# lab-emi/CleanUMamba

Hardware: AMD Instinct MI355X
Metric: audio samples/sec/node (train step, E8, 10s@16kHz) (higher is better)
Workload: dtype f16

## Files before the change

### cleanumamba_amd/csrc/gemm.hip

```cpp
#include <stdlib.h>
#include <type_traits>
#include "common.h"

namespace cum {

typedef __attribute__((ext_vector_type(8))) __bf16 bf16x8;
typedef __attribute__((ext_vector_type(8))) _Float16 f16x8;
typedef __attribute__((ext_vector_type(4))) float f32x4;
typedef __attribute__((ext_vector_type(4))) unsigned u32x4;

enum { EPI_BIAS = 0, EPI_RELU = 1, EPI_GLU = 2, EPI_MASK = 3, EPI_GLU_BWD = 4 };

struct GemmParams {
  const void *A, *W;
  const float *bias;
  const void *res;
  void *out;
  void *aux;
  const void *aux2;
  int64_t lda, ldw, ldc, ldr, ldz, ldy;
  int gate_only;
  int allow_split_k;
  int mask_bits;
  int M, N, K;
  int pitch, valid;
  int n_store;
  int64_t zero_head, zero_tail;
  int rows_epilogue;
  int group_m;
};

template <typename T>
struct Elem;
template <>
struct Elem<float> {
  static constexpr int EPC = 4;
  static __device__ __forceinline__ float to_f(float v) { return v; }
  static __device__ __forceinline__ float from_f(float v) { return v; }
};
template <>
struct Elem<__bf16> {
  static constexpr int EPC = 8;
  static __device__ __forceinline__ float to_f(__bf16 v) { return (float)v; }
  static __device__ __forceinline__ __bf16 from_f(float v) { return (__bf16)v; }
};

template <>
struct Elem<f16> {
  static constexpr int EPC = 8;
  static __device__ __forceinline__ float to_f(f16 v) { return (float)v; }
  static __device__ __forceinline__ f16 from_f(float v) { return (f16)v; }
};

template <typename T>
// ... 815 lines not shown
    __builtin_amdgcn_s_setprio(0);
    asm volatile("s_waitcnt lgkmcnt(0)"
                 : "+v"(af[0][4]), "+v"(af[0][5]), "+v"(af[0][6]), "+v"(af[0][7]), "+v"(af[1][4]), "+v"(af[1][5]),
                   "+v"(af[1][6]), "+v"(af[1][7]) : : "memory");
    asm volatile("s_barrier" ::: "memory");
    const bool early = more && wr == 0, late = more && wr != 0;
    if (early) {
      CUM_STAGE(0, kt + 2, par);
      CUM_STAGE(1, kt + 2, par);
    }
    __builtin_amdgcn_s_setprio(1);
    CUM_QUAD(1, 0);
    __builtin_amdgcn_s_setprio(0);
    __builtin_amdgcn_sched_barrier(0);
    if (late) {
      CUM_STAGE(0, kt + 2, par);
      CUM_STAGE(1, kt + 2, par);
    }
    CUM_DSR(wf[0][0], w0, 4096);  CUM_DSR(wf[0][1], w0, 6144);  CUM_DSR(wf[1][0], w1, 4096);  CUM_DSR(wf[1][1], w1, 6144);
    asm volatile("s_waitcnt lgkmcnt(0)" : "+v"(wf[0][0]), "+v"(wf[0][1]), "+v"(wf[1][0]), "+v"(wf[1][1]) : : "memory");
    asm volatile("s_barrier" ::: "memory");
    if (early) {
      CUM_STAGE(2, kt + 2, par);
      CUM_STAGE(3, kt + 2, par);
    }
    __builtin_amdgcn_s_setprio(1);
    CUM_QUAD(1, 2);
    __builtin_amdgcn_s_setprio(0);
    __builtin_amdgcn_sched_barrier(0);
    if (late) {
      CUM_STAGE(2, kt + 2, par);
      CUM_STAGE(3, kt + 2, par);
    }
    __builtin_amdgcn_s_setprio(1);
    CUM_QUAD(0, 2);
    __builtin_amdgcn_s_setprio(0);
  }
#undef CUM_HALFQ
#undef CUM_DSR
#undef CUM_QUAD
#undef CUM_STAGE
  asm volatile("s_barrier" ::: "memory");
  nt_epilogue_any<T, EPI, 2, 1>(p, acc, bv, m0, n0, 2 * wr, wc, lane,
                                reinterpret_cast<unsigned char *>(lds_all) + wave * nt_rows_lds(EPI));
}

#endif

template <typename T, int EPI>
__global__ __launch_bounds__(512) void gemm_nt9_kernel(const GemmParams p) {
  static_assert(sizeof(T) == 2, "16-bit element types only");
  constexpr int EPC = 8, BK = 64;
  constexpr int UNIT = 128 * 8;
  __shared__ uint4 lds_all[2 * 4 * UNIT];

  const int tid = threadIdx.x, lane = tid & 63;
  const int wave = uniform(tid >> 6);
  const int wr = wave >> 2, wc = wave & 3;
  const int g = lane >> 4, r = lane & 15;
  const int NB = (p.N + 255) / 256;
  const int xcd = blockIdx.x & 7, local = blockIdx.x >> 3;
  const int per = p.group_m * NB, grp = local / per, within = local - grp * per;
  const int left = (int)gridDim.x / (8 * NB) - grp * p.group_m;
  const int gm = left < p.group_m ? left : p.group_m;
  const int m_tile = (grp * p.group_m + within % gm) * 8 + xcd;
  const int n0 = (within / gm) * 256;
  const int m0 = m_tile * 256;
  if (m0 >= p.M) return;
  if (blockIdx.x == 0) {
    T *o = static_cast<T *>(p.out);
    T *x = (EPI != EPI_GLU && EPI != EPI_GLU_BWD && !(EPI == EPI_RELU && p.mask_bits)) ? static_cast<T *>(p.aux) : nullptr;
    for (int64_t i = threadIdx.x; i < p.zero_head; i += 512) {
      o[-1 - i] = Elem<T>::from_f(0.f);
      if (x) x[-1 - i] = Elem<T>::from_f(0.f);
    }
    const int64_t tail0 = (int64_t)p.M * p.ldc, tailx = (int64_t)p.M * p.ldz;
    for (int64_t i = threadIdx.x; i < p.zero_tail; i += 512) {
      o[tail0 + i] = Elem<T>::from_f(0.f);
      if (x) x[tailx + i] = Elem<T>::from_f(0.f);
    }
  }
  const T *A = static_cast<const T *>(p.A);
  const T *W = static_cast<const T *>(p.W);
  const T *src[4][2];
#pragma unroll
  for (int u = 0; u < 4; ++u)
#pragma unroll
    for (int it = 0; it < 2; ++it) {
      const int pos = it * 512 + tid;
      const int row = pos >> 3, cphys = pos & 7;
      const int clog = cphys ^ (row & 7);
      if (u < 2) {
        int am = m0 + 128 * u + row;
        am = am < p.M ? am : p.M - 1;
        src[u][it] = A + (int64_t)am * p.lda + clog * EPC;
      } else {
        int wn_ = n0 + 128 * (u - 2) + row;
        wn_ = wn_ < p.N ? wn_ : p.N - 1;
        src[u][it] = W + (int64_t)wn_ * p.ldw + clog * EPC;
      }
    }
  typedef __attribute__((address_space(3))) void *lds_ptr;
  typedef const __attribute__((address_space(1))) void *glb_ptr;
#define CUM_STAGE(u, kt, par)                                                                                   \
  do {                                                                                                          \
    _Pragma("unroll") for (int it = 0; it < 2; ++it)                                                           \
      __builtin_amdgcn_global_load_lds((glb_ptr)(src[u][it] + (kt) * BK),                                      \
                                       (lds_ptr)(&lds_all[((par) * 4 + (u)) * UNIT + it * 512 + wave * 64]), 16, 0, 0); \
  } while (0)

  f32x4 acc[2][4][4];
#pragma unroll
  for (int h = 0; h < 2; ++h)
#pragma unroll
    for (int i = 0; i < 4; ++i)
#pragma unroll
      for (int j = 0; j < 4; ++j) acc[h][i][j] = f32x4{0.f, 0.f, 0.f, 0.f};
  float bv[4][4];
  nt_load_bias(p, n0, wc, g, bv);

  const int nk = p.K / BK;
#pragma unroll
  for (int u = 0; u < 4; ++u) CUM_STAGE(u, 0, 0);
  if (nk > 1) {
#pragma unroll
    for (int u = 0; u < 4; ++u) CUM_STAGE(u, 1, 1);
  }
  const unsigned lds0 = (unsigned)(uintptr_t)(lds_ptr)lds_all;
  unsigned aA[2], aW[2];
#pragma unroll
  for (int ks = 0; ks < 2; ++ks) {
    const int cl = ks * 4 + g;
    aA[ks] = lds0 + (unsigned)((wr * UNIT + r * 8 + (cl ^ (r & 7))) * 16);
    aW[ks] = lds0 + (unsigned)(((2 + (wc >> 1)) * UNIT + ((wc & 1) * 64 + r) * 8 + (cl ^ (r & 7))) * 16);
  }
#define CUM_DSR(dst, addr, off) asm volatile("ds_read_b128 %0, %1 offset:" #off : "=v"(dst) : "v"(addr) : "memory")
#ifdef CUM_NT9_TIMING_NO_W_READS
#define CUM_DSRW(dst, addr, off) asm volatile("" : "=v"(dst) : "v"(addr))
#else
#define CUM_DSRW(dst, addr, off) CUM_DSR(dst, addr, off)
#endif
#define CUM_BAR()                               \
  do {                                          \
    __builtin_amdgcn_sched_barrier(0);          \
    asm volatile("s_barrier" ::: "memory");     \
    __builtin_amdgcn_sched_barrier(0);          \
  } while (0)
#define CUM_HALFQ(h, nlo, ks)                                                                                  \
  do {                                                                                                         \
    _Pragma("unroll") for (int ni = 0; ni < 2; ++ni)                                                           \
      _Pragma("unroll") for (int mi = 0; mi < 4; ++mi) {                                                       \
        if constexpr (__is_same(T, f16))                                                                       \
          acc[h][(nlo) + ni][mi] = __builtin_amdgcn_mfma_f32_16x16x32_f16(                                     \
              __builtin_bit_cast(f16x8, wf[ks][ni]), __builtin_bit_cast(f16x8, af[ks][4 * (h) + mi]),          \
              acc[h][(nlo) + ni][mi], 0, 0, 0);                                                                \
        else                                                                                                   \
          acc[h][(nlo) + ni][mi] = __builtin_amdgcn_mfma_f32_16x16x32_bf16(                                    \
              __builtin_bit_cast(bf16x8, wf[ks][ni]), __builtin_bit_cast(bf16x8, af[ks][4 * (h) + mi]),        \
              acc[h][(nlo) + ni][mi], 0, 0, 0);                                                                \
      }                                                                                                        \
  } while (0)
#define CUM_QUAD(h, nlo)                 \
  do {                                   \
    __builtin_amdgcn_s_setprio(1);       \
    CUM_HALFQ(h, nlo, 0);                \
    CUM_HALFQ(h, nlo, 1);                \
    __builtin_amdgcn_s_setprio(0);       \
  } while (0)

  if (nk > 1) asm volatile("s_waitcnt vmcnt(8)" ::: "memory");
  else asm volatile("s_waitcnt vmcnt(0)" ::: "memory");
  CUM_BAR();
  if (wr != 0) CUM_BAR();
  u32x4 af[2][8], wf[2][2];
  for (int kt = 0; kt < nk; ++kt) {
    const int par = kt & 1;
    const unsigned pb = (unsigned)par * (4 * UNIT * 16);
    const unsigned a0 = aA[0] + pb, a1 = aA[1] + pb, w0 = aW[0] + pb, w1 = aW[1] + pb;
    const bool more1 = kt + 1 < nk, more2 = kt + 2 < nk;
    CUM_DSRW(wf[0][0], w0, 0);    CUM_DSRW(wf[0][1], w0, 2048);
    CUM_DSR(af[0][0], a0, 0);     CUM_DSR(af[0][1], a0, 2048);  CUM_DSR(af[0][2], a0, 4096);  CUM_DSR(af[0][3], a0, 6144);
    CUM_DSRW(wf[1][0], w1, 0);    CUM_DSRW(wf[1][1], w1, 2048);
    CUM_DSR(af[1][0], a1, 0);     CUM_DSR(af[1][1], a1, 2048);  CUM_DSR(af[1][2], a1, 4096);  CUM_DSR(af[1][3], a1, 6144);
    if (wr == 0 && kt >= 1 && more1) {
      CUM_STAGE(2, kt + 1, par ^ 1);
      CUM_STAGE(3, kt + 1, par ^ 1);
    }
    CUM_BAR();
    asm volatile("s_waitcnt lgkmcnt(0)"
                 : "+v"(wf[0][0]), "+v"(wf[0][1]), "+v"(wf[1][0]), "+v"(wf[1][1]), "+v"(af[0][0]), "+v"(af[0][1]),
                   "+v"(af[0][2]), "+v"(af[0][3]), "+v"(af[1][0]), "+v"(af[1][1]), "+v"(af[1][2]), "+v"(af[1][3]) : : "memory");
    CUM_QUAD(0, 0);
    CUM_BAR();
    CUM_DSR(af[0][4], a0, 8192);  CUM_DSR(af[0][5], a0, 10240); CUM_DSR(af[0][6], a0, 12288); CUM_DSR(af[0][7], a0, 14336);
    CUM_DSR(af[1][4], a1, 8192);  CUM_DSR(af[1][5], a1, 10240); CUM_DSR(af[1][6], a1, 12288); CUM_DSR(af[1][7], a1, 14336);
    CUM_BAR();
    asm volatile("s_waitcnt lgkmcnt(0)"
                 : "+v"(af[0][4]), "+v"(af[0][5]), "+v"(af[0][6]), "+v"(af[0][7]), "+v"(af[1][4]), "+v"(af[1][5]),
                   "+v"(af[1][6]), "+v"(af[1][7]) : : "memory");
    CUM_QUAD(1, 0);
    CUM_BAR();
    CUM_DSRW(wf[0][0], w0, 4096); CUM_DSRW(wf[0][1], w0, 6144); CUM_DSRW(wf[1][0], w1, 4096); CUM_DSRW(wf[1][1], w1, 6144);
    if (more2) {
      CUM_STAGE(0, kt + 2, par);
      if (wr != 0) CUM_STAGE(1, kt + 2, par);
    }
    CUM_BAR();
    asm volatile("s_waitcnt lgkmcnt(0)" : "+v"(wf[0][0]), "+v"(wf[0][1]), "+v"(wf[1][0]), "+v"(wf[1][1]) : : "memory");
    CUM_QUAD(1, 2);
    CUM_BAR();
    if (wr == 0) {
      if (more2) CUM_STAGE(1, kt + 2, par);
    } else {
      if (more1) {
        if (more2) asm volatile("s_waitcnt vmcnt(4)" ::: "memory");
        else asm volatile("s_waitcnt vmcnt(0)" ::: "memory");
      }
      if (more2) {
        CUM_STAGE(2, kt + 2, par);
        CUM_STAGE(3, kt + 2, par);
      }
    }
    CUM_BAR();
    CUM_QUAD(0, 2);
    if (wr == 0 && more1) {
      if (more2) asm volatile("s_waitcnt vmcnt(4)" ::: "memory");
      else asm volatile("s_waitcnt vmcnt(0)" ::: "memory");
    }
    CUM_BAR();
  }
  if (wr == 0) CUM_BAR();
#undef CUM_HALFQ
#undef CUM_DSRW
#undef CUM_DSR
#undef CUM_QUAD
#undef CUM_STAGE
#undef CUM_BAR
  asm volatile("s_barrier" ::: "memory");
  nt_epilogue_any<T, EPI, 2, 1>(p, acc, bv, m0, n0, 2 * wr, wc, lane,
                                reinterpret_cast<unsigned char *>(lds_all) + wave * nt_rows_lds(EPI));
}

template <typename T, int EPI>
__global__ __launch_bounds__(512) void gemm_nt_ring_kernel(const GemmParams p) {
  static_assert(sizeof(T) == 2, "16-bit element types only");
#ifndef CUM_RING_NST
#define CUM_RING_NST 3
#endif
  constexpr int EPC = 8, BK = 64, BM = 128, BN = 256, NST = CUM_RING_NST;
  static_assert(NST == 2 || NST == 3, "two or three stages");
  constexpr int STAGE = (BM + BN) * 8;
  __shared__ uint4 lds_all[NST * STAGE];

  const int tid = threadIdx.x, lane = tid & 63;
  const int wave = uniform(tid >> 6);
  const int wm = wave >> 2, wn = wave & 3;
  const int g = lane >> 4, r = lane & 15;
  const int NB = (p.N + BN - 1) / BN;
  const int xcd = blockIdx.x & 7, local = blockIdx.x >> 3;
  const int m_tile = (local / NB) * 8 + xcd;
  const int n0 = (local % NB) * BN;
  const int m0 = m_tile * BM;
  if (m0 >= p.M) return;
  if (blockIdx.x == 0) {
    T *o = static_cast<T *>(p.out);
    T *x = (EPI != EPI_GLU && EPI != EPI_GLU_BWD && !(EPI == EPI_RELU && p.mask_bits)) ? static_cast<T *>(p.aux) : nullptr;
    for (int64_t i = threadIdx.x; i < p.zero_head; i += 512) {
      o[-1 - i] = Elem<T>::from_f(0.f);
      if (x) x[-1 - i] = Elem<T>::from_f(0.f);
    }
    const int64_t tail0 = (int64_t)p.M * p.ldc, tailx = (int64_t)p.M * p.ldz;
    for (int64_t i = threadIdx.x; i < p.zero_tail; i += 512) {
      o[tail0 + i] = Elem<T>::from_f(0.f);
      if (x) x[tailx + i] = Elem<T>::from_f(0.f);
    }
  }
  const T *A = static_cast<const T *>(p.A);
  const T *W = static_cast<const T *>(p.W);
  const T *ga[2], *gw[4];
#pragma unroll
  for (int it = 0; it < 2; ++it) {
    const int pos = it * 512 + tid, row = pos >> 3, clog = (pos & 7) ^ (row & 7);
    int am = m0 + row;
    am = am < p.M ? am : p.M - 1;
    ga[it] = A + (int64_t)am * p.lda + clog * EPC;
  }
#pragma unroll
  for (int it = 0; it < 4; ++it) {
    const int pos = it * 512 + tid, row = pos >> 3, clog = (pos & 7) ^ (row & 7);
    int wr = n0 + row;
    wr = wr < p.N ? wr : p.N - 1;
    gw[it] = W + (int64_t)wr * p.ldw + clog * EPC;
  }
// ... 441 lines not shown
  const int64_t total = M * ncol4;
  for (int64_t i = blockIdx.x * (int64_t)blockDim.x + threadIdx.x; i < total; i += (int64_t)gridDim.x * blockDim.x) {
    const int c = (i % ncol4) * 4;
    const int64_t m = i / ncol4;
    float y[4], d[4];
    load4<T>(Y + m * ldy + c, y);
    load4<T>(dO + m * ldo + c, d);
#pragma unroll
    for (int j = 0; j < 4; ++j) d[j] = y[j] > 0.f ? d[j] : 0.f;
    store4<T>(dZ + m * ldz + c, d);
  }
}

template <typename T>
__global__ void colsum_stage1(const T *__restrict__ X, int64_t M, int n, int64_t ld, int rows_per_block,
                              float *__restrict__ part) {
  const int c = blockIdx.x * blockDim.x + threadIdx.x;
  if (c >= n) return;
  const int64_t r0 = (int64_t)blockIdx.y * rows_per_block;
  int64_t r1 = r0 + rows_per_block;
  r1 = r1 < M ? r1 : M;
  float s = 0.f;
  for (int64_t m = r0; m < r1; ++m) s += Elem<T>::to_f(X[m * ld + c]);
  part[(int64_t)blockIdx.y * n + c] = s;
}
__global__ void colsum_stage2(const float *__restrict__ part, int nparts, int n, float *__restrict__ out) {
  const int c = blockIdx.x * blockDim.x + threadIdx.x;
  if (c >= n) return;
  float s = 0.f;
  for (int i = 0; i < nparts; ++i) s += part[(int64_t)i * n + c];
  out[c] = s;
}

#ifdef CUM_AB
template <typename T>
static int launch_gemm_nt8(const GemmParams &p, int epi, hipStream_t st) {
  if constexpr (sizeof(T) == 2) {
    const int NB = (p.N + 255) / 256, MB = (p.M + 255) / 256;
    dim3 grid(8 * NB * ((MB + 7) / 8)), block(512);
    switch (epi) {
      case EPI_BIAS: hipLaunchKernelGGL((gemm_nt8_kernel<T, EPI_BIAS>), grid, block, 0, st, p); break;
      case EPI_RELU: hipLaunchKernelGGL((gemm_nt8_kernel<T, EPI_RELU>), grid, block, 0, st, p); break;
      case EPI_MASK: hipLaunchKernelGGL((gemm_nt8_kernel<T, EPI_MASK>), grid, block, 0, st, p); break;
      case EPI_GLU_BWD: hipLaunchKernelGGL((gemm_nt8_kernel<T, EPI_GLU_BWD>), grid, block, 0, st, p); break;
      default: hipLaunchKernelGGL((gemm_nt8_kernel<T, EPI_GLU>), grid, block, 0, st, p); break;
    }
    CUM_CHECK_LAUNCH();
  }
  return CUM_OK;
}

#endif

template <typename T>
static int launch_gemm_nt9(const GemmParams &p0, int epi, hipStream_t st) {
  if constexpr (sizeof(T) == 2) {
    GemmParams p = p0;
    const int NB = (p.N + 255) / 256, MB = (p.M + 255) / 256;
    dim3 grid(8 * NB * ((MB + 7) / 8)), block(512);
    p.group_m = (int)cum_knob("CUM_NT_GROUPM", NB >= 24 ? 4 : 1);
    if (p.group_m < 1) p.group_m = 1;
#ifdef CUM_AB
#ifdef CUM_NT4_ONLY_BIAS
    if (cum_knob("CUM_NT4", 0) != 0 && epi == EPI_BIAS) {
      hipLaunchKernelGGL((gemm_nt4_kernel<T, EPI_BIAS>), grid, dim3(256), 0, st, p);
      CUM_CHECK_LAUNCH();
      return CUM_OK;
    }
#else
    if (cum_knob("CUM_NT4", 0) != 0) {
      const dim3 b4(256);
      switch (epi) {
        case EPI_BIAS: hipLaunchKernelGGL((gemm_nt4_kernel<T, EPI_BIAS>), grid, b4, 0, st, p); break;
        case EPI_RELU: hipLaunchKernelGGL((gemm_nt4_kernel<T, EPI_RELU>), grid, b4, 0, st, p); break;
        case EPI_MASK: hipLaunchKernelGGL((gemm_nt4_kernel<T, EPI_MASK>), grid, b4, 0, st, p); break;
        case EPI_GLU_BWD: hipLaunchKernelGGL((gemm_nt4_kernel<T, EPI_GLU_BWD>), grid, b4, 0, st, p); break;
        default: hipLaunchKernelGGL((gemm_nt4_kernel<T, EPI_GLU>), grid, b4, 0, st, p); break;
      }
      CUM_CHECK_LAUNCH();
      return CUM_OK;
    }
#endif
#endif
    switch (epi) {
      case EPI_BIAS: hipLaunchKernelGGL((gemm_nt9_kernel<T, EPI_BIAS>), grid, block, 0, st, p); break;
      case EPI_RELU: hipLaunchKernelGGL((gemm_nt9_kernel<T, EPI_RELU>), grid, block, 0, st, p); break;
      case EPI_MASK: hipLaunchKernelGGL((gemm_nt9_kernel<T, EPI_MASK>), grid, block, 0, st, p); break;
      case EPI_GLU_BWD: hipLaunchKernelGGL((gemm_nt9_kernel<T, EPI_GLU_BWD>), grid, block, 0, st, p); break;
      default: hipLaunchKernelGGL((gemm_nt9_kernel<T, EPI_GLU>), grid, block, 0, st, p); break;
    }
    CUM_CHECK_LAUNCH();
  }
  return CUM_OK;
}

template <typename T>
static int launch_gemm_ring(const GemmParams &p, int epi, hipStream_t st) {
  if constexpr (sizeof(T) == 2) {
    const int NB = (p.N + 255) / 256, MB = (p.M + 127) / 128;
    dim3 grid(8 * NB * ((MB + 7) / 8)), block(512);
    switch (epi) {
      case EPI_BIAS: hipLaunchKernelGGL((gemm_nt_ring_kernel<T, EPI_BIAS>), grid, block, 0, st, p); break;
      case EPI_RELU: hipLaunchKernelGGL((gemm_nt_ring_kernel<T, EPI_RELU>), grid, block, 0, st, p); break;
      case EPI_MASK: hipLaunchKernelGGL((gemm_nt_ring_kernel<T, EPI_MASK>), grid, block, 0, st, p); break;
      case EPI_GLU_BWD: hipLaunchKernelGGL((gemm_nt_ring_kernel<T, EPI_GLU_BWD>), grid, block, 0, st, p); break;
      default: hipLaunchKernelGGL((gemm_nt_ring_kernel<T, EPI_GLU>), grid, block, 0, st, p); break;
    }
    CUM_CHECK_LAUNCH();
  }
  return CUM_OK;
}

template <typename T, int BM, int BN>
static int launch_gemm_tile(const GemmParams &p, int epi, hipStream_t st) {
  const int NB = (p.N + BN - 1) / BN, MB = (p.M + BM - 1) / BM;
  dim3 grid(8 * NB * ((MB + 7) / 8)), block(BM * BN / 64);
  switch (epi) {
    case EPI_BIAS: hipLaunchKernelGGL((gemm_nt_kernel<T, EPI_BIAS, BM, BN>), grid, block, 0, st, p); break;
    case EPI_RELU: hipLaunchKernelGGL((gemm_nt_kernel<T, EPI_RELU, BM, BN>), grid, block, 0, st, p); break;
    case EPI_MASK: hipLaunchKernelGGL((gemm_nt_kernel<T, EPI_MASK, BM, BN>), grid, block, 0, st, p); break;
    case EPI_GLU_BWD: hipLaunchKernelGGL((gemm_nt_kernel<T, EPI_GLU_BWD, BM, BN>), grid, block, 0, st, p); break;
    default: hipLaunchKernelGGL((gemm_nt_kernel<T, EPI_GLU, BM, BN>), grid, block, 0, st, p); break;
  }
  CUM_CHECK_LAUNCH();
  return CUM_OK;
}

static int choose_tile(const GemmParams &p, int esz) {
  const int64_t mb256 = (p.M + 255) / 256;
  const int64_t tiles_256x256 = mb256 * ((p.N + 255) / 256), tiles_256x128 = mb256 * ((p.N + 127) / 128);
// ... 39 lines not shown
  } else {
    if (tile == 256) return launch_gemm_tile<T, 256, 128>(p, epi, st);
    return launch_gemm_tile<T, 128, 128>(p, epi, st);
  }
}

}

using namespace cum;

extern "C" int cum_gemm_nt(const cum_gemm_desc *d, const void *A, const void *W, const float *bias, const void *res,
                           void *out, void *aux, const void *aux2, void *stream) {
  CUM_REQUIRE(d && A && W && out, "gemm: null argument");
  CUM_REQUIRE(dtype_ok(d->dtype), "gemm: dtype must be CUM_F32, CUM_BF16 or CUM_F16");
  CUM_REQUIRE(d->epilogue >= 0 && d->epilogue <= 4, "gemm: bad epilogue");
  CUM_REQUIRE(d->epilogue != EPI_MASK || res, "gemm: the MASK epilogue needs the gating activation in res");
  CUM_REQUIRE(d->epilogue != EPI_GLU_BWD || (aux && d->zero_head == 0 && d->zero_tail == 0),
              "gemm: the GLU_BWD epilogue needs Z in aux and writes no framing rows");
  const int bk = is16(d->dtype) ? 64 : 32;
  const int epc = is16(d->dtype) ? 8 : 4;
  CUM_REQUIRE(d->M >= 0 && d->N > 0 && d->K > 0 && d->K % bk == 0, "gemm: K must be a positive multiple of the K tile");
  CUM_REQUIRE(d->N % (d->epilogue == 2 ? 32 : 16) == 0, "gemm: N must be a multiple of 16 (32 for GLU)");
  CUM_REQUIRE(d->lda % epc == 0 && d->ldw % epc == 0, "gemm: lda/ldw must keep rows 16-byte aligned");
  CUM_REQUIRE(d->ldc % 4 == 0 && d->ldr % 4 == 0 && d->ldz % 4 == 0 && d->n_store % 4 == 0, "gemm: ldc/ldr/ldz/n_store must be multiples of 4");
  CUM_REQUIRE(d->pitch > 0 && d->valid >= 0 && d->zero_head >= 0 && d->zero_tail >= 0, "gemm: bad pitch/valid/zero ranges");
  CUM_REQUIRE(((uintptr_t)A & 15) == 0 && ((uintptr_t)W & 15) == 0 && ((uintptr_t)bias & 15) == 0,
              "gemm: A, W and bias must be 16-byte aligned");
  if (d->M == 0) return CUM_OK;
  GemmParams p{};
  CUM_REQUIRE(!d->gate_only || d->epilogue == EPI_GLU || (d->epilogue == EPI_GLU_BWD && aux2 && d->ldy % 4 == 0),
              "gemm: gate_only applies to the GLU epilogues; GLU_BWD then needs the saved output in aux2");
  p.A = A; p.W = W; p.bias = bias; p.res = res; p.out = out; p.aux = aux; p.aux2 = aux2;
  p.lda = d->lda; p.ldw = d->ldw; p.ldc = d->ldc; p.ldr = d->ldr; p.ldz = d->ldz; p.ldy = d->ldy;
  p.gate_only = d->gate_only;
  p.mask_bits = d->mask_bits;
  p.allow_split_k = d->allow_split_k;
  CUM_REQUIRE(!d->mask_bits || (d->epilogue == EPI_RELU && aux) || d->epilogue == EPI_MASK,
              "gemm: mask_bits applies to RELU (aux = sign array) and MASK (res = sign array)");
  p.M = d->M; p.N = d->N; p.K = d->K; p.pitch = d->pitch; p.valid = d->valid; p.n_store = d->n_store;
  p.zero_head = d->zero_head; p.zero_tail = d->zero_tail;
  p.rows_epilogue = (int)cum_knob("CUM_NT8_ROWS", 1);
  if (d->dtype == CUM_BF16) return launch_gemm<__bf16>(p, d->epilogue, (hipStream_t)stream);
  if (d->dtype == CUM_F16) return launch_gemm<f16>(p, d->epilogue, (hipStream_t)stream);
  return launch_gemm<float>(p, d->epilogue, (hipStream_t)stream);
}

extern "C" int cum_gemm_nt_tile(const cum_gemm_desc *d) {
  CUM_REQUIRE(d && dtype_ok(d->dtype), "gemm_nt_tile: bad argument");
  GemmParams p{};
  p.M = d->M; p.N = d->N; p.K = d->K; p.allow_split_k = d->allow_split_k;
  return choose_tile(p, is16(d->dtype) ? 2 : 4);
}

extern "C" int cum_glu_bwd_gate(int32_t dtype, int64_t M, int32_t n_groups, int32_t n_out, const void *Bg, int64_t ldb,
                                const void *Y, int64_t ldy, const void *dOut, int64_t ldo, void *dZ, int64_t ldz,
                                void *stream) {
  CUM_REQUIRE(Bg && Y && dOut && dZ && n_groups > 0 && M >= 0, "glu_bwd_gate: bad argument");
  CUM_REQUIRE(ldb % 4 == 0 && ldy % 4 == 0 && ldo % 4 == 0 && ldz % 4 == 0, "glu_bwd_gate: strides must be multiples of 4");
  if (M == 0) return CUM_OK;
  const int64_t total = M * n_groups * 4;
  int blocks = (int)((total + 255) / 256 < 8192 ? (total + 255) / 256 : 8192);
  if (dtype == CUM_BF16)
    hipLaunchKernelGGL(glu_bwd_gate_kernel<__bf16>, dim3(blocks), dim3(256), 0, (hipStream_t)stream, (const __bf16 *)Bg,
                       (const __bf16 *)Y, (const __bf16 *)dOut, (__bf16 *)dZ, M, n_groups, ldb, ldy, ldo, ldz, n_out);
  else if (dtype == CUM_F16)
    hipLaunchKernelGGL(glu_bwd_gate_kernel<f16>, dim3(blocks), dim3(256), 0, (hipStream_t)stream, (const f16 *)Bg,
                       (const f16 *)Y, (const f16 *)dOut, (f16 *)dZ, M, n_groups, ldb, ldy, ldo, ldz, n_out);
  else
    hipLaunchKernelGGL(glu_bwd_gate_kernel<float>, dim3(blocks), dim3(256), 0, (hipStream_t)stream, (const float *)Bg,
                       (const float *)Y, (const float *)dOut, (float *)dZ, M, n_groups, ldb, ldy, ldo, ldz, n_out);
  CUM_CHECK_LAUNCH();
  return CUM_OK;
}

extern "C" int cum_glu_bwd(int32_t dtype, int64_t M, int32_t n_groups, int32_t n_out, const void *Z, int64_t ldz,
                           const void *dOut, int64_t ldo, void *dZ, void *stream) {
  CUM_REQUIRE(Z && dOut && dZ && n_groups > 0 && M >= 0, "glu_bwd: bad argument");
  CUM_REQUIRE(ldz % 4 == 0 && ldo % 4 == 0, "glu_bwd: strides must be multiples of 4");
  if (M == 0) return CUM_OK;
  const int64_t total = M * n_groups * 4;
  int blocks = (int)((total + 255) / 256 < 8192 ? (total + 255) / 256 : 8192);
  if (dtype == CUM_BF16)
    hipLaunchKernelGGL(glu_bwd_kernel<__bf16>, dim3(blocks), dim3(256), 0, (hipStream_t)stream, (const __bf16 *)Z,
                       (const __bf16 *)dOut, (__bf16 *)dZ, M, n_groups, ldz, ldo, n_out);
  else if (dtype == CUM_F16)
    hipLaunchKernelGGL(glu_bwd_kernel<f16>, dim3(blocks), dim3(256), 0, (hipStream_t)stream, (const f16 *)Z,
                       (const f16 *)dOut, (f16 *)dZ, M, n_groups, ldz, ldo, n_out);
  else
    hipLaunchKernelGGL(glu_bwd_kernel<float>, dim3(blocks), dim3(256), 0, (hipStream_t)stream, (const float *)Z,
                       (const float *)dOut, (float *)dZ, M, n_groups, ldz, ldo, n_out);
  CUM_CHECK_LAUNCH();
  return CUM_OK;
}

extern "C" int cum_relu_bwd(int32_t dtype, int64_t M, int32_t n_cols, const void *Y, int64_t ldy, const void *dOut,
                            int64_t ldo, void *dZ, int64_t ldz, int64_t zero_head, int64_t zero_tail, void *stream) {
  CUM_REQUIRE(Y && dOut && dZ && n_cols > 0 && n_cols % 4 == 0 && M >= 0, "relu_bwd: bad argument");
  CUM_REQUIRE(ldy % 4 == 0 && ldo % 4 == 0 && ldz % 4 == 0, "relu_bwd: strides must be multiples of 4");
  if (M == 0) return CUM_OK;
  const int64_t total = M * (n_cols / 4);
  int blocks = (int)((total + 255) / 256 < 8192 ? (total + 255) / 256 : 8192);
  if (dtype == CUM_BF16)
    hipLaunchKernelGGL(relu_bwd_kernel<__bf16>, dim3(blocks), dim3(256), 0, (hipStream_t)stream, (const __bf16 *)Y,
                       (const __bf16 *)dOut, (__bf16 *)dZ, M, n_cols / 4, ldy, ldo, ldz, zero_head, zero_tail);
  else if (dtype == CUM_F16)
    hipLaunchKernelGGL(relu_bwd_kernel<f16>, dim3(blocks), dim3(256), 0, (hipStream_t)stream, (const f16 *)Y,
// ... 35 lines not shown
```

### cleanumamba_amd/hip.py

```python
import ctypes
import os

import torch

_HERE = os.path.dirname(os.path.abspath(__file__))
LIB_PATH = os.environ.get("CUM_LIB") or os.path.join(_HERE, "libcleanumamba_hip.so")

c_i32, c_i64, c_f32p, c_vp = ctypes.c_int32, ctypes.c_int64, ctypes.c_void_p, ctypes.c_void_p


class ScanShape(ctypes.Structure):
    _fields_ = [("batch", c_i32), ("dim", c_i32), ("dstate", c_i32), ("len", c_i32),
                ("u_sb", c_i64), ("u_sd", c_i64), ("u_sl", c_i64),
                ("dt_sb", c_i64), ("dt_sd", c_i64), ("dt_sl", c_i64),
                ("z_sb", c_i64), ("z_sd", c_i64), ("z_sl", c_i64),
                ("o_sb", c_i64), ("o_sd", c_i64), ("o_sl", c_i64),
                ("B_sb", c_i64), ("B_sn", c_i64), ("B_sl", c_i64),
                ("C_sb", c_i64), ("C_sn", c_i64), ("C_sl", c_i64),
                ("delta_softplus", c_i32), ("io_dtype", c_i32)]


class ScanGradStrides(ctypes.Structure):
    _fields_ = [("du_sb", c_i64), ("du_sd", c_i64), ("du_sl", c_i64),
                ("dd_sb", c_i64), ("dd_sd", c_i64), ("dd_sl", c_i64),
# ... 15 lines not shown


class GemmDesc(ctypes.Structure):
    _fields_ = [("dtype", c_i32), ("epilogue", c_i32), ("M", c_i32), ("N", c_i32), ("K", c_i32),
                ("lda", c_i64), ("ldw", c_i64), ("ldc", c_i64), ("ldr", c_i64), ("ldz", c_i64),
                ("pitch", c_i32), ("valid", c_i32), ("n_store", c_i32), ("zero_head", c_i64), ("zero_tail", c_i64),
                ("gate_only", c_i32), ("ldy", c_i64), ("mask_bits", c_i32), ("allow_split_k", c_i32)]


class PruneImpDesc(ctypes.Structure):
    _fields_ = [("w", ctypes.c_void_p), ("g", ctypes.c_void_p), ("numel", c_i64), ("off", c_i64), ("ch_stride", c_i64),
                ("head_stride", c_i64), ("s0", c_i64), ("s1", c_i64), ("channels", c_i32), ("heads", c_i32),
                ("n0", c_i32), ("n1", c_i32), ("out", c_i64), ("lanes_on_channels", c_i32), ("pad_", c_i32)]


class PruneGatherDesc(ctypes.Structure):
    _fields_ = [("src", c_i64), ("dst", c_i64), ("n_new", c_i64), ("ndim", c_i32), ("old_dims", c_i32 * 3),
                ("new_dims", c_i32 * 3), ("pad_", c_i32), ("keep", c_i64 * 3)]


class PruneMaskDesc(ctypes.Structure):
    _fields_ = [("w", ctypes.c_void_p), ("numel", c_i64), ("row_stride", c_i64), ("s0", c_i64), ("s1", c_i64),
                ("n0", c_i32), ("n1", c_i32), ("rows", c_i32), ("n_rows", c_i32), ("first", c_i64),
                ("rows_fastest", c_i32), ("pad_", c_i32)]


CUM_F32, CUM_BF16, CUM_F16 = 0, 1, 2
HALF_TYPES = (torch.bfloat16, torch.float16)
IO_TYPES = (torch.float32,) + HALF_TYPES
EPI_BIAS, EPI_RELU, EPI_GLU, EPI_MASK, EPI_GLU_BWD = 0, 1, 2, 3, 4

_P = ctypes.c_void_p
SIGNATURES = {
    "cum_abi_version": (c_i32, []),
    "cum_last_error": (ctypes.c_char_p, []),
    "cum_scan_chunk": (c_i32, []),
    "cum_scan_ckpt_elems": (c_i64, [c_i32, c_i32, c_i32, c_i32]),
    "cum_selective_scan_fwd": (c_i32, [ctypes.POINTER(ScanShape)] + [_P] * 12),
    "cum_scan_fwd_workspace_elems": (c_i64, [c_i32, c_i32, c_i32, c_i32]),
    "cum_selective_scan_fwd_ws": (c_i32, [ctypes.POINTER(ScanShape)] + [_P] * 14),
    "cum_scan_fwd_keeps_y": (c_i32, [c_i32, c_i32, c_i32, c_i32, c_i32]),
    "cum_scan_bwd_workspace_elems": (c_i64, [c_i32, c_i32, c_i32, c_i32]),
    "cum_selective_scan_bwd": (c_i32, [ctypes.POINTER(ScanShape), ctypes.POINTER(ScanGradStrides)] + [_P] * 21),
    "cum_scan_bwd_tp_workspace_elems": (c_i64, [c_i32, c_i32, c_i32, c_i32]),
    "cum_selective_scan_bwd_tp": (c_i32, [ctypes.POINTER(ScanShape), ctypes.POINTER(ScanGradStrides)] + [_P] * 21),
    "cum_selective_state_update": (c_i32, [c_i32, c_i32, c_i32, _P, _P, _P, _P, _P, c_i64, _P, c_i64,
                                           _P, _P, _P, c_i32, _P, _P]),
    "cum_causal_conv1d_fwd": (c_i32, [ctypes.POINTER(ConvShape)] + [_P] * 5),
    "cum_conv_bwd_workspace_elems": (c_i64, [c_i32, c_i32, c_i32, c_i32]),
    "cum_causal_conv1d_bwd": (c_i32, [ctypes.POINTER(ConvShape)] + [_P] * 5 + [c_i64] * 3 + [_P] * 4),
    "cum_causal_conv1d_update": (c_i32, [c_i32, c_i32, c_i32, _P, _P, _P, _P, c_i32, _P, _P]),
    "cum_gemm_nt": (c_i32, [ctypes.POINTER(GemmDesc)] + [_P] * 8),
    "cum_gemm_nt_tile": (c_i32, [ctypes.POINTER(GemmDesc)]),
    "cum_gemm_tn_tile": (c_i32, [c_i32, c_i64, c_i32, c_i32]),
    "cum_glu_bwd_gate": (c_i32, [c_i32, c_i64, c_i32, c_i32, _P, c_i64, _P, c_i64, _P, c_i64, _P, c_i64, _P]),
    "cum_glu_bwd": (c_i32, [c_i32, c_i64, c_i32, c_i32, _P, c_i64, _P, c_i64, _P, _P]),
    "cum_relu_bwd": (c_i32, [c_i32, c_i64, c_i32, _P, c_i64, _P, c_i64, _P, c_i64, c_i64, c_i64, _P]),
    "cum_colsum_workspace_elems": (c_i64, [c_i64, c_i32]),
    "cum_colsum": (c_i32, [c_i32, c_i64, c_i32, _P, c_i64, _P, _P, _P]),
    "cum_gemm_tn_workspace_elems": (c_i64, [c_i32, c_i64, c_i32, c_i32]),
    "cum_gemm_tn": (c_i32, [c_i32, c_i64, c_i32, c_i32, _P, c_i64, _P, c_i64, _P, c_i64, _P, _P, _P]),
    "cum_stft_frames": (c_i32, [_P, c_i64, c_i64, c_i64, c_i32, c_i32, c_i32, _P, _P, c_i64, _P]),
    "cum_stft_loss_workspace_elems": (c_i64, [c_i64, c_i64]),
    "cum_stft_loss_fwd": (c_i32, [_P, _P, c_i64, c_i64, c_i32, c_i64, _P, _P, _P]),
    "cum_stft_loss_bwd": (c_i32, [_P, _P, c_i64, c_i64, c_i32, c_i64, _P, _P, _P, _P, _P]),
    "cum_stft_fold": (c_i32, [_P, c_i64, c_i64, c_i32, c_i32, c_i32, _P, c_i64, _P, c_i64, c_i32, _P]),
    "cum_gather": (c_i32, [c_i32, _P, _P, c_i64, c_i32, _P, _P]),
    "cum_pack2d": (c_i32, [_P, _P, _P, c_i32, _P, c_i32, _P, _P]),
    "cum_add_layernorm_fwd": (c_i32, [c_i32, c_i32, c_i64, c_i32, c_i32, _P, c_i64, c_i64, _P, _P, _P, ctypes.c_float,
                                      _P, _P, _P, _P, _P]),
    "cum_add_layernorm_bwd_workspace_elems": (c_i64, [c_i32]),
    "cum_add_layernorm_bwd": (c_i32, [c_i32, c_i32, c_i64, c_i32] + [_P] * 12),
    "cum_small_linear": (c_i32, [c_i32, c_i32, c_i32, _P, c_i64, _P, _P, _P, c_i64, _P]),
    "cum_mamba_step_supported": (c_i32, [c_i32] * 5),
    "cum_mamba_step": (c_i32, [c_i32] * 6 + [ctypes.c_float] + [_P] * 20),
    "cum_stream_window_update": (c_i32, [c_i32, c_i32, c_i32, c_i32, c_i32, _P, _P, c_i64, c_i64, c_i32, _P, _P, c_i64, _P]),
    "cum_stream_tail_rows": (c_i32, [c_i32, c_i32, c_i32, c_i32, _P, c_i64, c_i32, _P, c_i64, _P]),
    "cum_stream_overlap_add": (c_i32, [c_i32, c_i32, c_i32, c_i32, c_i32, _P, c_i64, _P, _P, _P, c_i64, _P, c_i64, c_i32, _P]),
    "cum_stream_hop_plan_ints": (c_i32, []),
    "cum_stream_hop_max_lds_bytes": (c_i32, []),
    "cum_stream_hop": (c_i32, [_P, _P, _P, c_i64, c_i32, _P, c_i64, _P, c_i64, c_i32, c_i32, _P]),
    "cum_stream_hop_slots": (c_i32, [_P, _P, _P, c_i64, c_i32, _P, _P, c_i32, _P, c_i64, _P, c_i64, c_i32, _P]),
    "cum_stream_pool_stage": (c_i32, [_P, c_i64, c_i32, _P, _P, c_i32, _P, c_i64, _P, c_i64, _P]),
    "cum_fft_plan_create": (c_i32, [c_i32, c_i32, c_i64, ctypes.POINTER(ctypes.c_void_p), ctypes.POINTER(c_i64)]),
    "cum_fft_plan_destroy": (c_i32, [_P]),
    "cum_fft_exec": (c_i32, [_P, _P, _P, c_i32, _P, _P]),
    "cum_stft_fused_supported": (c_i32, [c_i32]),
    "cum_stft_fused_workspace_elems": (c_i64, [c_i64, c_i64]),
    "cum_stft_fused_fwd": (c_i32, [_P, _P, c_i64, c_i64, c_i64, c_i64, c_i32, c_i32, c_i32, _P, _P, c_i64, c_i64, _P, _P, _P]),
    "cum_stft_fused_bwd": (c_i32, [_P, _P, c_i64, c_i64, c_i64, c_i64, c_i32, c_i32, c_i32, _P, _P, c_i64, c_i64, _P, _P, _P,
                                   _P, _P]),
    "cum_stft_loss_fwd_packed": (c_i32, [_P, _P, c_i64, c_i64, c_i32, c_i64, _P, _P, _P, _P]),
    "cum_stft_loss_bwd_packed": (c_i32, [_P, _P, c_i64, c_i64, c_i32, c_i64, _P, _P, _P, _P, _P, _P]),
    "cum_enc0_fwd": (c_i32, [c_i32, c_i64, c_i32, c_i32, _P, _P, _P, _P, _P, _P, c_i64, _P, _P]),
    "cum_ench_fwd": (c_i32, [c_i32, c_i64, c_i32, c_i32, _P, c_i64, _P, _P, _P, _P, _P, c_i64, _P, _P, c_i64, _P, _P]),
    "cum_dech_fwd": (c_i32, [c_i32, c_i64, c_i32, c_i32, _P, c_i64, _P, _P, _P, _P, _P, _P, c_i64, _P, _P, c_i64, _P, _P]),
    "cum_enc0_bwd_workgroups": (c_i32, [c_i64]),
    "cum_enc0_bwd_workspace_elems": (c_i64, [c_i64]),
    "cum_enc0_bwd": (c_i32, [c_i32, c_i64, c_i32, c_i32, _P, _P, _P, _P, _P, _P, _P, _P, _P]),
    "cum_dec7_fwd": (c_i32, [c_i32, c_i64, c_i32, c_i32, _P, _P, _P, _P, _P, _P, c_i64, _P]),
    "cum_dec7_bwd_workgroups": (c_i32, [c_i64]),
    "cum_dec7_bwd_workspace_elems": (c_i64, [c_i64]),
    "cum_dec7_bwd": (c_i32, [c_i32, c_i64, c_i32, c_i32, _P, _P, _P, _P, _P, _P, _P, _P, c_i64, _P, _P, _P, _P]),
    "cum_lp_loss_parts": (c_i32, [c_i64]),
    "cum_lp_loss_fwd": (c_i32, [c_i32, _P, _P, c_i64, _P, _P, _P]),
    "cum_lp_loss_bwd": (c_i32, [c_i32, _P, _P, c_i64, _P, _P, _P]),
# ... 144 lines not shown
```

### include/cleanumamba_hip.h

```cpp
#ifndef CLEANUMAMBA_HIP_H
#define CLEANUMAMBA_HIP_H

#include <stdint.h>

#ifdef __cplusplus
extern "C" {
#endif

#define CUM_OK 0
#define CUM_EINVAL (-1)
#define CUM_ELAUNCH (-2)
#define CUM_EWORKSPACE (-3)

#define CUM_ABI_VERSION 16

int cum_abi_version(void);
const char *cum_last_error(void);

int cum_scan_chunk(void);

#define CUM_SCAN_SOFTPLUS 1
#define CUM_SCAN_A_IS_LOG 2
typedef struct {
  int32_t batch, dim, dstate, len;
// ... 45 lines not shown
                              const float *ckpt, void *du, void *ddelta, float *dA, float *dB,
                              float *dC, float *dD, void *dz, float *ddelta_bias,
                              float *workspace, void *stream);

int cum_selective_state_update(int32_t batch, int32_t dim, int32_t dstate, float *state,
                               const float *x, const float *dt, const float *A,
                               const float *Bv, int64_t B_sb, const float *Cv, int64_t C_sb,
                               const float *D, const float *z, const float *dt_bias,
                               int32_t dt_softplus, float *out, void *stream);

typedef struct {
  int32_t batch, dim, len, width;
  int64_t x_sb, x_sd, x_sl;
  int64_t y_sb, y_sd, y_sl;
  int32_t silu;
  int32_t io_dtype;
} cum_conv_shape;

int cum_causal_conv1d_fwd(const cum_conv_shape *s, const void *x, const float *weight,
                          const float *bias, void *y, void *stream);

int64_t cum_conv_bwd_workspace_elems(int32_t batch, int32_t dim, int32_t len, int32_t width);

int cum_causal_conv1d_bwd(const cum_conv_shape *s, const void *x, const float *weight,
                          const float *bias, const void *dy, void *dx, int64_t dx_sb,
                          int64_t dx_sd, int64_t dx_sl, float *dweight, float *dbias,
                          float *workspace, void *stream);

int cum_causal_conv1d_update(int32_t batch, int32_t dim, int32_t width, float *conv_state,
                             const float *x, const float *weight, const float *bias,
                             int32_t silu, float *y, void *stream);

#define CUM_F32 0
#define CUM_BF16 1
#define CUM_F16 2

typedef struct {
  int32_t dtype, epilogue;
  int32_t M, N, K;
  int64_t lda, ldw, ldc, ldr, ldz;
  int32_t pitch, valid;
  int32_t n_store;
  int64_t zero_head;
  int64_t zero_tail;
  int32_t gate_only;
  int64_t ldy;
  int32_t mask_bits;
  int32_t allow_split_k;
} cum_gemm_desc;

int cum_gemm_nt(const cum_gemm_desc *d, const void *A, const void *W, const float *bias,
                const void *res, void *out, void *aux, const void *aux2, void *stream);
int cum_gemm_nt_tile(const cum_gemm_desc *d);

int cum_glu_bwd(int32_t dtype, int64_t M, int32_t n_groups, int32_t n_out, const void *Z,
                int64_t ldz, const void *dOut, int64_t ldo, void *dZ, void *stream);
int cum_glu_bwd_gate(int32_t dtype, int64_t M, int32_t n_groups, int32_t n_out, const void *Bg,
                     int64_t ldb, const void *Y, int64_t ldy, const void *dOut, int64_t ldo, void *dZ,
                     int64_t ldz, void *stream);

int cum_relu_bwd(int32_t dtype, int64_t M, int32_t n_cols, const void *Y, int64_t ldy,
                 const void *dOut, int64_t ldo, void *dZ, int64_t ldz, int64_t zero_head,
                 int64_t zero_tail, void *stream);

int64_t cum_colsum_workspace_elems(int64_t M, int32_t n_cols);
int cum_colsum(int32_t dtype, int64_t M, int32_t n_cols, const void *X, int64_t ld, float *out,
               float *workspace, void *stream);

int64_t cum_gemm_tn_workspace_elems(int32_t dtype, int64_t M, int32_t N, int32_t K);
int cum_gemm_tn(int32_t dtype, int64_t M, int32_t N, int32_t K, const void *dZ, int64_t ldz,
                const void *X, int64_t ldx, float *dW, int64_t ldw, float *db, float *workspace,
                void *stream);
int cum_gemm_tn_tile(int32_t dtype, int64_t M, int32_t N, int32_t K);

int cum_stft_frames(const float *x, int64_t batch, int64_t len, int64_t x_stride_b, int32_t n_fft, int32_t hop,
                    int32_t win_length, const float *window, float *frames, int64_t n_frames, void *stream);
int64_t cum_stft_loss_workspace_elems(int64_t batch, int64_t n_frames);
int cum_stft_loss_fwd(const float *spec_x, const float *spec_y, int64_t batch, int64_t n_frames, int32_t bins,
                      int64_t frame0, float *workspace, float *stats, void *stream);
int cum_stft_loss_bwd(const float *spec_x, const float *spec_y, int64_t batch, int64_t n_frames, int32_t bins,
                      int64_t frame0, const float *stats, const float *g_sc, const float *g_mag, float *zspec,
                      void *stream);
int cum_stft_fold(const float *dframes, int64_t batch, int64_t len, int32_t n_fft, int32_t hop, int32_t win_length,
                  const float *window, int64_t n_frames, float *dx, int64_t dx_stride_b, int32_t accumulate,
                  void *stream);

int cum_gather(int32_t src_dtype, const void *src, const int32_t *idx, int64_t n, int32_t dst_dtype, void *dst,
               void *stream);

int cum_pack2d(const float *src, const void *jobs, const int32_t *tiles, int32_t n_tiles, const int32_t *tables,
               int32_t dst_dtype, void *dst, void *stream);

int cum_fft_plan_create(int32_t kind, int32_t n, int64_t batch, void **plan, int64_t *work_bytes);
int cum_fft_plan_destroy(void *plan);
int cum_fft_exec(void *plan, float *in, float *out, int32_t inverse, void *work, void *stream);

int cum_stft_loss_fwd_packed(const float *zx, const float *zy, int64_t batch, int64_t n_frames, int32_t n_fft,
                             int64_t frame0, const float *twiddle, float *workspace, float *stats, void *stream);
int cum_stft_loss_bwd_packed(const float *zx, const float *zy, int64_t batch, int64_t n_frames, int32_t n_fft,
                             int64_t frame0, const float *stats, const float *g_sc, const float *g_mag,
                             const float *twiddle, float *gz, void *stream);

int cum_stft_fused_supported(int32_t n_fft);
int64_t cum_stft_fused_workspace_elems(int64_t batch, int64_t n_frames);
int cum_stft_fused_fwd(const float *x, const float *y, int64_t batch, int64_t len, int64_t x_stride_b,
                       int64_t y_stride_b, int32_t n_fft, int32_t hop, int32_t win_length, const float *window,
// ... 178 lines not shown
```

Before: 137.7 million.

## Make nt9 GEMM persistent with one workgroup per CU and overlapped epilogue

Converts the nt9 GEMM kernel into a persistent kernel. The grid is capped at the device CU count, and each workgroup walks a contiguous range of 256x256 tiles while keeping the XCD-aware grouped ordering. The next tile's first K-stage global-to-LDS loads are issued before the current tile's epilogue runs. Epilogue staging moves into a dedicated extra LDS region so those prefetches do not overwrite it. This aims to cut launch and tail overhead and hide epilogue time, at the cost of more LDS per workgroup, possible load imbalance across tiles, and a new grid-cap API.

```diff
diff --git a/cleanumamba_amd/csrc/gemm.hip b/cleanumamba_amd/csrc/gemm.hip
--- a/cleanumamba_amd/csrc/gemm.hip
+++ b/cleanumamba_amd/csrc/gemm.hip
@@ -1,5 +1,6 @@
 #include <stdlib.h>
 #include <type_traits>
+#include <algorithm>
 #include "common.h"
 
 namespace cum {
@@ -921,21 +922,30 @@
   static_assert(sizeof(T) == 2, "16-bit element types only");
   constexpr int EPC = 8, BK = 64;
   constexpr int UNIT = 128 * 8;
-  __shared__ uint4 lds_all[2 * 4 * UNIT];
+  __shared__ uint4 lds_all[2 * 4 * UNIT + 2 * UNIT];
+  static_assert(8 * nt_rows_lds(EPI) <= (4 * UNIT + 2 * UNIT) * 16, "epilogue staging must fit beside ring stage 0");
 
   const int tid = threadIdx.x, lane = tid & 63;
   const int wave = uniform(tid >> 6);
   const int wr = wave >> 2, wc = wave & 3;
   const int g = lane >> 4, r = lane & 15;
-  const int NB = (p.N + 255) / 256;
-  const int xcd = blockIdx.x & 7, local = blockIdx.x >> 3;
-  const int per = p.group_m * NB, grp = local / per, within = local - grp * per;
-  const int left = (int)gridDim.x / (8 * NB) - grp * p.group_m;
-  const int gm = left < p.group_m ? left : p.group_m;
-  const int m_tile = (grp * p.group_m + within % gm) * 8 + xcd;
-  const int n0 = (within / gm) * 256;
-  const int m0 = m_tile * 256;
-  if (m0 >= p.M) return;
+  const int NB = (p.N + 255) / 256, MB = (p.M + 255) / 256;
+  const int G = (int)gridDim.x, nx = G >= 8 ? 8 : 1;
+  const int xcd = (int)blockIdx.x & (nx - 1), local = (int)blockIdx.x / nx;
+  const int wgs = (G - xcd + nx - 1) / nx;
+  const int ms = (MB - xcd + nx - 1) / nx;
+  const int ntiles = ms * NB;
+  int t = local * (ntiles / wgs) + min(local, ntiles % wgs);
+  const int t_end = t + ntiles / wgs + (local < ntiles % wgs ? 1 : 0);
+  int m0, n0;
+  auto tile_origin = [&](int tt, int &tm0, int &tn0) {
+    const int per = p.group_m * NB, grp = tt / per, within = tt - grp * per;
+    const int left = ms - grp * p.group_m;
+    const int gm = left < p.group_m ? left : p.group_m;
+    const int q = within / gm;
+    tm0 = ((grp * p.group_m + within - q * gm) * nx + xcd) * 256;
+    tn0 = q * 256;
+  };
   if (blockIdx.x == 0) {
     T *o = static_cast<T *>(p.out);
     T *x = (EPI != EPI_GLU && EPI != EPI_GLU_BWD && !(EPI == EPI_RELU && p.mask_bits)) ? static_cast<T *>(p.aux) : nullptr;
@@ -949,26 +959,33 @@
       if (x) x[tailx + i] = Elem<T>::from_f(0.f);
     }
   }
+  if (t >= t_end) return;
   const T *A = static_cast<const T *>(p.A);
   const T *W = static_cast<const T *>(p.W);
   const T *src[4][2];
-#pragma unroll
-  for (int u = 0; u < 4; ++u)
-#pragma unroll
-    for (int it = 0; it < 2; ++it) {
-      const int pos = it * 512 + tid;
-      const int row = pos >> 3, cphys = pos & 7;
-      const int clog = cphys ^ (row & 7);
-      if (u < 2) {
-        int am = m0 + 128 * u + row;
-        am = am < p.M ? am : p.M - 1;
-        src[u][it] = A + (int64_t)am * p.lda + clog * EPC;
-      } else {
-        int wn_ = n0 + 128 * (u - 2) + row;
-        wn_ = wn_ < p.N ? wn_ : p.N - 1;
-        src[u][it] = W + (int64_t)wn_ * p.ldw + clog * EPC;
-      }
-    }
+  auto tile_sources = [&](int tm0, int tn0) {
+    int tid_ = tid;
+    asm volatile("" : "+v"(tid_));
+#pragma unroll
+    for (int u = 0; u < 4; ++u)
+#pragma unroll
+      for (int it = 0; it < 2; ++it) {
+        const int pos = it * 512 + tid_;
+        const int row = pos >> 3, cphys = pos & 7;
+        const int clog = cphys ^ (row & 7);
+        if (u < 2) {
+          int am = tm0 + 128 * u + row;
+          am = am < p.M ? am : p.M - 1;
+          src[u][it] = A + (int64_t)am * p.lda + clog * EPC;
+        } else {
+          int wn_ = tn0 + 128 * (u - 2) + row;
+          wn_ = wn_ < p.N ? wn_ : p.N - 1;
+          src[u][it] = W + (int64_t)wn_ * p.ldw + clog * EPC;
+        }
+      }
+  };
+  tile_origin(t, m0, n0);
+  tile_sources(m0, n0);
   typedef __attribute__((address_space(3))) void *lds_ptr;
   typedef const __attribute__((address_space(1))) void *glb_ptr;
 #define CUM_STAGE(u, kt, par)                                                                                   \
@@ -979,12 +996,6 @@
   } while (0)
 
   f32x4 acc[2][4][4];
-#pragma unroll
-  for (int h = 0; h < 2; ++h)
-#pragma unroll
-    for (int i = 0; i < 4; ++i)
-#pragma unroll
-      for (int j = 0; j < 4; ++j) acc[h][i][j] = f32x4{0.f, 0.f, 0.f, 0.f};
   float bv[4][4];
   nt_load_bias(p, n0, wc, g, bv);
 
@@ -997,12 +1008,6 @@
   }
   const unsigned lds0 = (unsigned)(uintptr_t)(lds_ptr)lds_all;
   unsigned aA[2], aW[2];
-#pragma unroll
-  for (int ks = 0; ks < 2; ++ks) {
-    const int cl = ks * 4 + g;
-    aA[ks] = lds0 + (unsigned)((wr * UNIT + r * 8 + (cl ^ (r & 7))) * 16);
-    aW[ks] = lds0 + (unsigned)(((2 + (wc >> 1)) * UNIT + ((wc & 1) * 64 + r) * 8 + (cl ^ (r & 7))) * 16);
-  }
 #define CUM_DSR(dst, addr, off) asm volatile("ds_read_b128 %0, %1 offset:" #off : "=v"(dst) : "v"(addr) : "memory")
 #ifdef CUM_NT9_TIMING_NO_W_READS
 #define CUM_DSRW(dst, addr, off) asm volatile("" : "=v"(dst) : "v"(addr))
@@ -1037,6 +1042,25 @@
     __builtin_amdgcn_s_setprio(0);       \
   } while (0)
 
+  unsigned char *const stage_lds = reinterpret_cast<unsigned char *>(lds_all) + 4 * UNIT * 16 + wave * nt_rows_lds(EPI);
+  for (;;) {
+#pragma unroll
+  for (int h = 0; h < 2; ++h)
+#pragma unroll
+    for (int i = 0; i < 4; ++i)
+#pragma unroll
+      for (int j = 0; j < 4; ++j) acc[h][i][j] = f32x4{0.f, 0.f, 0.f, 0.f};
+  {
+    int lane_ = lane;
+    asm volatile("" : "+v"(lane_));
+    const int g_ = lane_ >> 4, r_ = lane_ & 15;
+#pragma unroll
+    for (int ks = 0; ks < 2; ++ks) {
+      const int cl = ks * 4 + g_;
+      aA[ks] = lds0 + (unsigned)((wr * UNIT + r_ * 8 + (cl ^ (r_ & 7))) * 16);
+      aW[ks] = lds0 + (unsigned)(((2 + (wc >> 1)) * UNIT + ((wc & 1) * 64 + r_) * 8 + (cl ^ (r_ & 7))) * 16);
+    }
+  }
   if (nk > 1) asm volatile("s_waitcnt vmcnt(8)" ::: "memory");
   else asm volatile("s_waitcnt vmcnt(0)" ::: "memory");
   CUM_BAR();
@@ -1099,15 +1123,39 @@
     CUM_BAR();
   }
   if (wr == 0) CUM_BAR();
+  asm volatile("s_barrier" ::: "memory");
+  const int em0 = m0, en0 = n0;
+  const bool more = ++t < t_end;
+  if (more) {
+    tile_origin(t, m0, n0);
+    tile_sources(m0, n0);
+#pragma unroll
+    for (int u = 0; u < 4; ++u) CUM_STAGE(u, 0, 0);
+  }
+  {
+    int lane_ = lane;
+    asm volatile("" : "+v"(lane_));
+    nt_epilogue_any<T, EPI, 2, 1>(p, acc, bv, em0, en0, 2 * wr, wc, lane_, stage_lds);
+  }
+  if (!more) break;
+  asm volatile("s_waitcnt lgkmcnt(0)\n\ts_barrier" ::: "memory");
+  tile_sources(m0, n0);
+  {
+    int lane_ = lane;
+    asm volatile("" : "+v"(lane_));
+    nt_load_bias(p, n0, wc, lane_ >> 4, bv);
+  }
+  if (nk > 1) {
+#pragma unroll
+    for (int u = 0; u < 4; ++u) CUM_STAGE(u, 1, 1);
+  }
+  }
 #undef CUM_HALFQ
 #undef CUM_DSRW
 #undef CUM_DSR
 #undef CUM_QUAD
 #undef CUM_STAGE
 #undef CUM_BAR
-  asm volatile("s_barrier" ::: "memory");
-  nt_epilogue_any<T, EPI, 2, 1>(p, acc, bv, m0, n0, 2 * wr, wc, lane,
-                                reinterpret_cast<unsigned char *>(lds_all) + wave * nt_rows_lds(EPI));
 }
 
 template <typename T, int EPI>
@@ -1655,18 +1703,39 @@
 
 #endif
 
+static int g_nt9_grid_cap = 0;
+
+static int device_cus() {
+  static int cus[64];
+  int dev = 0;
+  if (hipGetDevice(&dev) != hipSuccess || dev < 0 || dev >= 64) return 0;
+  if (cus[dev] == 0) {
+    int n = 0;
+    if (hipDeviceGetAttribute(&n, hipDeviceAttributeMultiprocessorCount, dev) != hipSuccess) return 0;
+    cus[dev] = n;
+  }
+  return cus[dev];
+}
+
 template <typename T>
 static int launch_gemm_nt9(const GemmParams &p0, int epi, hipStream_t st) {
   if constexpr (sizeof(T) == 2) {
     GemmParams p = p0;
     const int NB = (p.N + 255) / 256, MB = (p.M + 255) / 256;
-    dim3 grid(8 * NB * ((MB + 7) / 8)), block(512);
+    const int cus = device_cus();
+    CUM_REQUIRE(cus > 0, "gemm: cannot read the device's CU count");
+    int64_t wgs = std::min<int64_t>((int64_t)NB * MB, cus);
+    if (g_nt9_grid_cap > 0) wgs = std::min<int64_t>(wgs, g_nt9_grid_cap);
+    dim3 grid((unsigned)wgs), block(512);
+#ifdef CUM_AB
+    const dim3 grid4(8 * NB * ((MB + 7) / 8));
+#endif
     p.group_m = (int)cum_knob("CUM_NT_GROUPM", NB >= 24 ? 4 : 1);
     if (p.group_m < 1) p.group_m = 1;
 #ifdef CUM_AB
 #ifdef CUM_NT4_ONLY_BIAS
     if (cum_knob("CUM_NT4", 0) != 0 && epi == EPI_BIAS) {
-      hipLaunchKernelGGL((gemm_nt4_kernel<T, EPI_BIAS>), grid, dim3(256), 0, st, p);
+      hipLaunchKernelGGL((gemm_nt4_kernel<T, EPI_BIAS>), grid4, dim3(256), 0, st, p);
       CUM_CHECK_LAUNCH();
       return CUM_OK;
     }
@@ -1674,11 +1743,11 @@
     if (cum_knob("CUM_NT4", 0) != 0) {
       const dim3 b4(256);
       switch (epi) {
-        case EPI_BIAS: hipLaunchKernelGGL((gemm_nt4_kernel<T, EPI_BIAS>), grid, b4, 0, st, p); break;
-        case EPI_RELU: hipLaunchKernelGGL((gemm_nt4_kernel<T, EPI_RELU>), grid, b4, 0, st, p); break;
-        case EPI_MASK: hipLaunchKernelGGL((gemm_nt4_kernel<T, EPI_MASK>), grid, b4, 0, st, p); break;
-        case EPI_GLU_BWD: hipLaunchKernelGGL((gemm_nt4_kernel<T, EPI_GLU_BWD>), grid, b4, 0, st, p); break;
-        default: hipLaunchKernelGGL((gemm_nt4_kernel<T, EPI_GLU>), grid, b4, 0, st, p); break;
+        case EPI_BIAS: hipLaunchKernelGGL((gemm_nt4_kernel<T, EPI_BIAS>), grid4, b4, 0, st, p); break;
+        case EPI_RELU: hipLaunchKernelGGL((gemm_nt4_kernel<T, EPI_RELU>), grid4, b4, 0, st, p); break;
+        case EPI_MASK: hipLaunchKernelGGL((gemm_nt4_kernel<T, EPI_MASK>), grid4, b4, 0, st, p); break;
+        case EPI_GLU_BWD: hipLaunchKernelGGL((gemm_nt4_kernel<T, EPI_GLU_BWD>), grid4, b4, 0, st, p); break;
+        default: hipLaunchKernelGGL((gemm_nt4_kernel<T, EPI_GLU>), grid4, b4, 0, st, p); break;
       }
       CUM_CHECK_LAUNCH();
       return CUM_OK;
@@ -1824,6 +1893,12 @@
   return choose_tile(p, is16(d->dtype) ? 2 : 4);
 }
 
+extern "C" int cum_gemm_nt_set_grid_cap(int workgroups) {
+  CUM_REQUIRE(workgroups >= 0, "gemm_nt_set_grid_cap: the cap is a workgroup count, 0 = one per CU");
+  g_nt9_grid_cap = workgroups;
+  return CUM_OK;
+}
+
 extern "C" int cum_glu_bwd_gate(int32_t dtype, int64_t M, int32_t n_groups, int32_t n_out, const void *Bg, int64_t ldb,
                                 const void *Y, int64_t ldy, const void *dOut, int64_t ldo, void *dZ, int64_t ldz,
                                 void *stream) {
diff --git a/cleanumamba_amd/hip.py b/cleanumamba_amd/hip.py
--- a/cleanumamba_amd/hip.py
+++ b/cleanumamba_amd/hip.py
@@ -91,6 +91,7 @@
     "cum_causal_conv1d_update": (c_i32, [c_i32, c_i32, c_i32, _P, _P, _P, _P, c_i32, _P, _P]),
     "cum_gemm_nt": (c_i32, [ctypes.POINTER(GemmDesc)] + [_P] * 8),
     "cum_gemm_nt_tile": (c_i32, [ctypes.POINTER(GemmDesc)]),
+    "cum_gemm_nt_set_grid_cap": (c_i32, [c_i32]),
     "cum_gemm_tn_tile": (c_i32, [c_i32, c_i64, c_i32, c_i32]),
     "cum_glu_bwd_gate": (c_i32, [c_i32, c_i64, c_i32, c_i32, _P, c_i64, _P, c_i64, _P, c_i64, _P, c_i64, _P]),
     "cum_glu_bwd": (c_i32, [c_i32, c_i64, c_i32, c_i32, _P, c_i64, _P, c_i64, _P, _P]),
diff --git a/include/cleanumamba_hip.h b/include/cleanumamba_hip.h
--- a/include/cleanumamba_hip.h
+++ b/include/cleanumamba_hip.h
@@ -121,6 +121,7 @@
 int cum_gemm_nt(const cum_gemm_desc *d, const void *A, const void *W, const float *bias,
                 const void *res, void *out, void *aux, const void *aux2, void *stream);
 int cum_gemm_nt_tile(const cum_gemm_desc *d);
+int cum_gemm_nt_set_grid_cap(int workgroups);
 
 int cum_glu_bwd(int32_t dtype, int64_t M, int32_t n_groups, int32_t n_out, const void *Z,
                 int64_t ldz, const void *dOut, int64_t ldo, void *dZ, void *stream);
```

New measurement: 135.2 million. 0.982x the previous value.
